# PinataFarms/FEARTracker

Measured on NVIDIA H100. Metric: FEAR-XS frames/sec (track + decode, batch 256 per GPU), higher is better.
Workload: dtype f32

## Files before the change

### feartracker_b200/csrc/kernels_tc.cuh

```cuda
#pragma once
#include <cuda_runtime.h>
#include <stdlib.h>

#include <initializer_list>

#include "tc_common.cuh"

namespace fear {
namespace tc {

constexpr int kCorrChunk = 32;
constexpr int kCorrABytes = 128 * 128;
constexpr int kCorrBBytes = 64 * 128;
constexpr int kTcThreads = 288;
constexpr int kTcConsumers = 256;

__device__ __forceinline__ void consumer_sync() { asm volatile("bar.sync 1, 256;" ::: "memory"); }

constexpr int kCorrStages = 3;
constexpr int kCorrStageBytes = kCorrABytes + 2 * kCorrBBytes;
constexpr int kCorrSmemBytes = kCorrStages * kCorrStageBytes + 1024  + 256 ;

__global__ void __launch_bounds__(kTcThreads, 1)
corr_tc_kernel(const __grid_constant__ CUtensorMap tmA, const __grid_constant__ CUtensorMap tmB,
               float* __restrict__ cat, int z_mod) {
  extern __shared__ uint8_t smem_raw[];
  uint8_t* smem = smem_raw + ((1024u - (smem_u32(smem_raw) & 1023u)) & 1023u);
  uint64_t* full = reinterpret_cast<uint64_t*>(smem + kCorrStages * kCorrStageBytes);
  uint64_t* empty = full + kCorrStages;
  const int warp = threadIdx.x >> 5, lane = threadIdx.x & 31;
  constexpr int kChunks = 256 / kCorrChunk;
  if (threadIdx.x == 0) {
    prefetch_tmap(&tmA);
    prefetch_tmap(&tmB);
    for (int s = 0; s < kCorrStages; ++s) {
      mbar_init(&full[s], 1);
      mbar_init(&empty[s], 8);
    }
    fence_mbar_init();
  }
  __syncthreads();
  pdl_trigger();
  pdl_wait();
  const int frame = blockIdx.x >> 1, half = blockIdx.x & 1;
  const int arow = frame * 256 + half * 128;
  auto st_x = [&](int s) { return smem + s * kCorrStageBytes; };
  auto st_z = [&](int s) { return smem + s * kCorrStageBytes + kCorrABytes; };

  if (warp == 8) {
    if (lane == 0) {
      const int brow = z_mod ? (frame % z_mod) * 64 : 0;
      for (int c = 0; c < kChunks; ++c) {
        const int stage = c % kCorrStages;
        mbar_wait_backoff(&empty[stage], (uint32_t)(((c / kCorrStages) & 1) ^ 1));
        mbar_arrive_expect_tx(&full[stage], kCorrABytes + kCorrBBytes);
        tma_load_2d(st_x(stage), &tmA, &full[stage], c * kCorrChunk, arow);
        tma_load_2d(st_z(stage), &tmB, &full[stage], c * kCorrChunk, brow);
      }
    }
    return;
  }
  const int wg = warp >> 2, r0 = wg * 64 + (warp & 3) * 16 + (lane >> 2), t = lane & 3;
  float accm[32], accc[32];
#pragma unroll
  for (int i = 0; i < 32; ++i) accm[i] = accc[i] = 0.f;
  for (int c = 0; c < kChunks; ++c) {
    const int stage = c % kCorrStages;
    mbar_wait(&full[stage], (uint32_t)((c / kCorrStages) & 1));
    float4* zh = reinterpret_cast<float4*>(st_z(stage));
    float4* zl = reinterpret_cast<float4*>(st_z(stage) + kCorrBBytes);
#pragma unroll
    for (int i = 0; i < kCorrBBytes / 16 / kTcConsumers; ++i) {
      const float4 v = zh[threadIdx.x + i * kTcConsumers];
      float4 h, l;
      split_tf32_trunc(v.x, h.x, l.x);
      split_tf32_trunc(v.y, h.y, l.y);
      split_tf32_trunc(v.z, h.z, l.z);
      split_tf32_trunc(v.w, h.w, l.w);
      zh[threadIdx.x + i * kTcConsumers] = h;
      zl[threadIdx.x + i * kTcConsumers] = l;
    }
    fence_proxy_async_smem();
    consumer_sync();
    uint32_t hi[4][4], lo[4][4];
    load_a_frags(st_x(stage), r0, t, hi, lo);
    const uint32_t bh = smem_u32(zh), bl = smem_u32(zl);
    wg_fence();
#pragma unroll
    for (int j = 0; j < 4; ++j) mma3<64>(accm, accc, hi[j], lo[j], bh + j * 32, bl + j * 32);
    wg_commit();
    wg_wait();
    __syncwarp();
    if (lane == 0) mbar_arrive(&empty[stage]);
  }
  float* out = cat + (long long)(arow + r0) * 320 + 256 + 2 * t;
#pragma unroll
  for (int i = 0; i < 8; ++i) {
    *reinterpret_cast<float2*>(out + 8 * i) = make_float2(accm[4 * i] + accc[4 * i], accm[4 * i + 1] + accc[4 * i + 1]);
    *reinterpret_cast<float2*>(out + 8 * 320 + 8 * i) =
        make_float2(accm[4 * i + 2] + accc[4 * i + 2], accm[4 * i + 3] + accc[4 * i + 3]);
  }
}

inline int init_pw();

inline int init() {
  int dev = 0;
  if (cudaGetDevice(&dev) != cudaSuccess) return -1;
  cudaDeviceProp p;
  if (cudaGetDeviceProperties(&p, dev) != cudaSuccess) return -1;
  DeviceState& st = dev_state();
  st.num_sms = p.multiProcessorCount;
  st.inited = true;
  if (resolve_driver()) return 0;
  if (cudaFuncSetAttribute(corr_tc_kernel, cudaFuncAttributeMaxDynamicSharedMemorySize, kCorrSmemBytes) != cudaSuccess) {
    cudaGetLastError();
    return 0;
  }
  if (init_pw()) return 0;
  st.tc_ready = true;
  return 0;
}

inline int launch_corr(cudaStream_t s, const float* zt, int Bz, float* cat, int B, int groups) {
  if (!available()) return -20;
  CUtensorMap tmA, tmB;
  const int frames = B * groups;
  int r;
  r = make_tmap_2d(&tmA, cat, (uint64_t)frames * 256, 320, 320, 128, kCorrChunk);
  if (r) return r;
  r = make_tmap_2d(&tmB, zt, (uint64_t)Bz * 64, 256, 256, 64, kCorrChunk);
  if (r) return r;
  if (launch_pdl(corr_tc_kernel, dim3(frames * 2), dim3(kTcThreads), kCorrSmemBytes, s, tmA, tmB, cat, Bz == 1 ? 0 : B) !=
      cudaSuccess)
    return -23;
  return 0;
}

struct PwParams {
  const float* bias;
  const float* R;
  float* C;
  int ldr, ldc;
  int M, N, num_n_tiles, num_tiles, num_chunks, last_ksteps, relu, stages, stage_bytes;
  int dw_relu, dw_bias;
  int box_bytes;
};

constexpr int kPwThreads = 384;
constexpr int kPwProducerRegs = 40, kPwConsumerRegs = 232;

template <int NT, int KS>
__device__ __forceinline__ void mma3_chunk(float* accm, float* accc, const uint32_t (&hi)[4][4], const uint32_t (&lo)[4][4],
                                           uint32_t bh, uint32_t bl) {
#pragma unroll
  for (int j = 0; j < KS; ++j) mma3<NT>(accm, accc, hi[j], lo[j], bh + j * 32, bl + j * 32);
}

template <int K, int MW>
__device__ __forceinline__ void dw_chunk(const uint8_t* box, const uint8_t* wts, const uint8_t* bia, uint8_t* at, int ct,
                                         int dw_bias, int dw_relu) {
  constexpr int TX = 8, NIN = TX + K - 1, IW = MW + K - 1, PXN = MW / TX;
  typedef unsigned long long U2;
  const int c2 = ct & 15, pos = ct >> 4;
  const int x0 = (pos % PXN) * TX, y0 = pos / PXN;
  const U2* in2 = reinterpret_cast<const U2*>(box) + (y0 * IW + x0) * 16 + c2;
  const U2* w2 = reinterpret_cast<const U2*>(wts) + c2;
  const U2 bias2 = dw_bias ? reinterpret_cast<const U2*>(bia)[c2] : 0ull;
  U2 acc[TX];
#pragma unroll
  for (int i = 0; i < TX; ++i) acc[i] = bias2;
#pragma unroll
  for (int ky = 0; ky < K; ++ky) {
    U2 v[NIN];
#pragma unroll
    for (int i = 0; i < NIN; ++i) v[i] = in2[(ky * IW + i) * 16];
#pragma unroll
    for (int kx = 0; kx < K; ++kx) {
      const U2 k = w2[(ky * K + kx) * 16];
#pragma unroll
      for (int i = 0; i < TX; ++i) ffma2(acc[i], v[i + kx], k);
    }
  }
#pragma unroll
  for (int i = 0; i < TX; ++i) {
    float2 v = make_float2(__uint_as_float((uint32_t)acc[i]), __uint_as_float((uint32_t)(acc[i] >> 32)));
    if (dw_relu) {
      v.x = fmaxf(v.x, 0.f);
      v.y = fmaxf(v.y, 0.f);
    }
    const int R = y0 * MW + x0 + i;
    *reinterpret_cast<float2*>(at + R * 128 + (((c2 >> 1) ^ (R & 7)) << 4) + ((c2 & 1) << 3)) = v;
  }
}

template <int NT>
__device__ __forceinline__ void pw_epilogue(const PwParams& p, const float* accm, const float* accc, int mt, int nt, int r0,
                                            int t) {
  const int n0 = nt * NT + 2 * t;
#pragma unroll
  for (int hrow = 0; hrow < 2; ++hrow) {
    const long long grow = (long long)mt * 128 + r0 + hrow * 8;
    if (grow >= p.M) continue;
#pragma unroll
    for (int i = 0; i < NT / 8; ++i) {
      const int col = n0 + 8 * i;
      if (col >= p.N) continue;
      float2 o = make_float2(accm[4 * i + 2 * hrow] + accc[4 * i + 2 * hrow], accm[4 * i + 2 * hrow + 1] + accc[4 * i + 2 * hrow + 1]);
      float2 b = p.bias ? __ldg(reinterpret_cast<const float2*>(p.bias + col)) : make_float2(0.f, 0.f);
      if (p.R) {
        const float2 rr = __ldg(reinterpret_cast<const float2*>(p.R + grow * p.ldr + col));
        b.x += rr.x;
        b.y += rr.y;
      }
      o.x += b.x;
      o.y += b.y;
      if (p.relu) {
        o.x = fmaxf(o.x, 0.f);
        o.y = fmaxf(o.y, 0.f);
      }
      *reinterpret_cast<float2*>(p.C + grow * p.ldc + col) = o;
    }
  }
}

template <int NT, int DWK, int MW = 16>
__global__ void __launch_bounds__(kPwThreads, 1)
pw_tc_kernel(const __grid_constant__ CUtensorMap tmA, const __grid_constant__ CUtensorMap tmWh,
             const __grid_constant__ CUtensorMap tmWl, const __grid_constant__ CUtensorMap tmDW,
             const __grid_constant__ CUtensorMap tmDB, const PwParams p) {
  extern __shared__ uint8_t smem_raw[];
  uint8_t* smem = smem_raw + ((1024u - (smem_u32(smem_raw) & 1023u)) & 1023u);
  const int S = p.stages;
  constexpr int a_bufs = DWK > 0 ? 2 : 0;
  uint64_t* full = reinterpret_cast<uint64_t*>(smem + S * p.stage_bytes + a_bufs * kCorrABytes);
  uint64_t* empty = full + S;
  constexpr int w_bytes = NT * 128;
  if (threadIdx.x == 0) {
    prefetch_tmap(&tmA);
    prefetch_tmap(&tmWh);
    prefetch_tmap(&tmWl);
    for (int s = 0; s < S; ++s) {
      mbar_init(&full[s], 1);
      mbar_init(&empty[s], 8);
    }
    fence_mbar_init();
  }
  __syncthreads();
  pdl_trigger();
  pdl_wait();

  auto a_tile = [&](int s) { return smem + s * p.stage_bytes; };
  auto a_buf = [&](int b) { return smem + S * p.stage_bytes + b * kCorrABytes; };
  auto w_hi = [&](int s) { return smem + s * p.stage_bytes + (DWK > 0 ? 0 : kCorrABytes); };
  auto w_lo = [&](int s) { return w_hi(s) + w_bytes; };
  auto dw_box = [&](int s) { return w_lo(s) + w_bytes; };
  auto dw_wts = [&](int s) { return dw_box(s) + p.box_bytes; };
  auto dw_bia = [&](int s) { return dw_wts(s) + DWK * DWK * 128; };

  const int wg = __shfl_sync(0xffffffffu, (int)threadIdx.x / 128, 0);
  if (wg == 0) {
    setmaxnreg_dec<kPwProducerRegs>();
    if (threadIdx.x == 0) {
      constexpr int th = 128 / MW, tpf = MW / th;
      int stage = 0;
      uint32_t phase = 0;
      for (int tile = blockIdx.x; tile < p.num_tiles; tile += gridDim.x) {
        const int mt = tile / p.num_n_tiles, nt = tile - mt * p.num_n_tiles;
        for (int c = 0; c < p.num_chunks; ++c) {
          mbar_wait_backoff(&empty[stage], phase ^ 1);
          if constexpr (DWK > 0) {
            mbar_arrive_expect_tx(&full[stage], 2 * w_bytes + p.box_bytes + DWK * DWK * 128 + (p.dw_bias ? 128 : 0));
            tma_load_4d(dw_box(stage), &tmA, &full[stage], c * 32, -(DWK / 2), (mt % tpf) * th - DWK / 2, mt / tpf);
            tma_load_2d(dw_wts(stage), &tmDW, &full[stage], c * 32, 0);
            if (p.dw_bias) tma_load_2d(dw_bia(stage), &tmDB, &full[stage], c * 32, 0);
          } else {
            mbar_arrive_expect_tx(&full[stage], kCorrABytes + 2 * w_bytes);
            tma_load_2d(a_tile(stage), &tmA, &full[stage], c * 32, mt * 128);
          }
          tma_load_2d(w_hi(stage), &tmWh, &full[stage], c * 32, nt * NT);
          tma_load_2d(w_lo(stage), &tmWl, &full[stage], c * 32, nt * NT);
          if (++stage == S) {
            stage = 0;
            phase ^= 1;
          }
        }
      }
    }
    return;
  }
  setmaxnreg_inc<kPwConsumerRegs>();

  const int ct = threadIdx.x - 128, warp = ct >> 5, lane = ct & 31;
  const int r0 = (warp >> 2) * 64 + (warp & 3) * 16 + (lane >> 2), t = lane & 3;
  int stage = 0, ab = 0;
  uint32_t phase = 0;
  for (int tile = blockIdx.x; tile < p.num_tiles; tile += gridDim.x) {
    const int mt = tile / p.num_n_tiles, nt = tile - mt * p.num_n_tiles;
    float accm[NT / 2], accc[NT / 2];
#pragma unroll
    for (int i = 0; i < NT / 2; ++i) accm[i] = accc[i] = 0.f;
    if constexpr (DWK > 0) {
      mbar_wait(&full[stage], phase);
      dw_chunk<DWK, MW>(dw_box(stage), dw_wts(stage), dw_bia(stage), a_buf(ab), ct, p.dw_bias, p.dw_relu);
      consumer_sync();
    }
    int prev = 0;
    for (int c = 0; c < p.num_chunks; ++c) {
      if constexpr (DWK == 0) mbar_wait(&full[stage], phase);
      uint32_t hi[4][4], lo[4][4];
      load_a_frags(DWK > 0 ? a_buf(ab) : a_tile(stage), r0, t, hi, lo);
      const uint32_t bh = smem_u32(w_hi(stage)), bl = smem_u32(w_lo(stage));
      const int ksteps = (c == p.num_chunks - 1) ? p.last_ksteps : 4;
      wg_fence();
      if (ksteps == 4) mma3_chunk<NT, 4>(accm, accc, hi, lo, bh, bl);
      else if (ksteps == 3) mma3_chunk<NT, 3>(accm, accc, hi, lo, bh, bl);
      else if (ksteps == 2) mma3_chunk<NT, 2>(accm, accc, hi, lo, bh, bl);
      else mma3_chunk<NT, 1>(accm, accc, hi, lo, bh, bl);
      wg_commit();
      if (c > 0) {
        wg_wait_n<1>();
        __syncwarp();
        if (lane == 0) mbar_arrive(&empty[prev]);
      }
      prev = stage;
      if (++stage == S) {
        stage = 0;
        phase ^= 1;
      }
      if constexpr (DWK > 0) {
        ab ^= 1;
        if (c + 1 < p.num_chunks) {
          mbar_wait(&full[stage], phase);
          dw_chunk<DWK, MW>(dw_box(stage), dw_wts(stage), dw_bia(stage), a_buf(ab), ct, p.dw_bias, p.dw_relu);
          consumer_sync();
        }
      }
    }
    wg_wait_n<0>();
    __syncwarp();
    if (lane == 0) mbar_arrive(&empty[prev]);
    pw_epilogue<NT>(p, accm, accc, mt, nt, r0, t);
  }
}

template <int NT>
__global__ void __launch_bounds__(kTcThreads, 1)
pw_tc_narrow_kernel(const __grid_constant__ CUtensorMap tmA, const __grid_constant__ CUtensorMap tmWh,
                    const __grid_constant__ CUtensorMap tmWl, const PwParams p) {
  extern __shared__ uint8_t smem_raw[];
  uint8_t* smem = smem_raw + ((1024u - (smem_u32(smem_raw) & 1023u)) & 1023u);
  const int S = p.stages;
  uint64_t* full = reinterpret_cast<uint64_t*>(smem + S * p.stage_bytes);
  uint64_t* empty = full + S;
  const int warp = threadIdx.x >> 5, lane = threadIdx.x & 31;
  constexpr int w_bytes = NT * 128;
  if (threadIdx.x == 0) {
    prefetch_tmap(&tmA);
    prefetch_tmap(&tmWh);
    prefetch_tmap(&tmWl);
    for (int s = 0; s < S; ++s) {
      mbar_init(&full[s], 1);
      mbar_init(&empty[s], 8);
    }
    fence_mbar_init();
  }
  __syncthreads();
  pdl_trigger();
  pdl_wait();

  const int mt = blockIdx.x / p.num_n_tiles, nt = blockIdx.x - mt * p.num_n_tiles;
  auto a_tile = [&](int s) { return smem + s * p.stage_bytes; };
  auto w_hi = [&](int s) { return smem + s * p.stage_bytes + kCorrABytes; };
  auto w_lo = [&](int s) { return w_hi(s) + w_bytes; };

  if (warp == 8) {
    if (lane == 0) {
      for (int c = 0; c < p.num_chunks; ++c) {
        const int stage = c % S;
        mbar_wait_backoff(&empty[stage], (uint32_t)(((c / S) & 1) ^ 1));
        mbar_arrive_expect_tx(&full[stage], kCorrABytes + 2 * w_bytes);
        tma_load_2d(a_tile(stage), &tmA, &full[stage], c * 32, mt * 128);
        tma_load_2d(w_hi(stage), &tmWh, &full[stage], c * 32, nt * NT);
        tma_load_2d(w_lo(stage), &tmWl, &full[stage], c * 32, nt * NT);
      }
    }
    return;
  }

  const int wg = warp >> 2, r0 = wg * 64 + (warp & 3) * 16 + (lane >> 2), t = lane & 3;
  float accm[NT / 2], accc[NT / 2];
#pragma unroll
  for (int i = 0; i < NT / 2; ++i) accm[i] = accc[i] = 0.f;
  for (int c = 0; c < p.num_chunks; ++c) {
    const int stage = c % S;
    mbar_wait(&full[stage], (uint32_t)((c / S) & 1));
    uint32_t hi[4][4], lo[4][4];
    load_a_frags(a_tile(stage), r0, t, hi, lo);
    const uint32_t bh = smem_u32(w_hi(stage)), bl = smem_u32(w_lo(stage));
    const int ksteps = (c == p.num_chunks - 1) ? p.last_ksteps : 4;
    wg_fence();
#pragma unroll
    for (int j = 0; j < 4; ++j)
      if (j < ksteps) mma3<NT>(accm, accc, hi[j], lo[j], bh + j * 32, bl + j * 32);
    wg_commit();
    wg_wait();
    __syncwarp();
    if (lane == 0) mbar_arrive(&empty[stage]);
  }
  pw_epilogue<NT>(p, accm, accc, mt, nt, r0, t);
}

constexpr int kPwMaxSmem = 232448 - 1024;
constexpr int kPwMaxStages = 4;
constexpr int kPwSmemExtra = 1024  + 256 ;

inline int pw_stages(int stage_bytes, int fixed_bytes) {
  const int fit = (kPwMaxSmem - kPwSmemExtra - fixed_bytes) / stage_bytes;
  return fit < kPwMaxStages ? fit : kPwMaxStages;
}

inline int pw_tile_n(int N) {
  const int Np = (N + 15) & ~15;
  const int tiles = (Np + 127) / 128;
  const int need = (Np + tiles - 1) / tiles;
  for (int nt : {16, 32, 48, 64, 96, 112, 128})
    if (nt >= need) return nt;
  return 0;
}

inline bool pw_supported(int cin, int cout) { return available() && cin % 8 == 0 && cout % 8 == 0; }

#define FEAR_PW_FOR_NT(X) X(16) X(32) X(48) X(64) X(96) X(112) X(128)

constexpr int kPwNarrowNT = 32;
inline int pw_tile_n_one_chunk(int N) {
  const int Np = (N + 15) & ~15;
  const int tiles = (Np + kPwNarrowNT - 1) / kPwNarrowNT;
  const int need = (Np + tiles - 1) / tiles;
  return need <= 16 ? 16 : 32;
}

inline int init_pw() {
  cudaError_t e = cudaSuccess;
#define FEAR_PW_ATTR(NT_)                                                                                                  \
  if (e == cudaSuccess) e = cudaFuncSetAttribute(pw_tc_kernel<NT_, 0>, cudaFuncAttributeMaxDynamicSharedMemorySize, kPwMaxSmem);     \
  if (e == cudaSuccess) e = cudaFuncSetAttribute(pw_tc_kernel<NT_, 3, 16>, cudaFuncAttributeMaxDynamicSharedMemorySize, kPwMaxSmem); \
  if (e == cudaSuccess) e = cudaFuncSetAttribute(pw_tc_kernel<NT_, 5, 16>, cudaFuncAttributeMaxDynamicSharedMemorySize, kPwMaxSmem); \
  if (e == cudaSuccess) e = cudaFuncSetAttribute(pw_tc_kernel<NT_, 3, 32>, cudaFuncAttributeMaxDynamicSharedMemorySize, kPwMaxSmem); \
  if (e == cudaSuccess) e = cudaFuncSetAttribute(pw_tc_kernel<NT_, 5, 32>, cudaFuncAttributeMaxDynamicSharedMemorySize, kPwMaxSmem);
  FEAR_PW_FOR_NT(FEAR_PW_ATTR)
#undef FEAR_PW_ATTR
  if (e == cudaSuccess) e = cudaFuncSetAttribute(pw_tc_narrow_kernel<16>, cudaFuncAttributeMaxDynamicSharedMemorySize, kPwMaxSmem);
  if (e == cudaSuccess) e = cudaFuncSetAttribute(pw_tc_narrow_kernel<32>, cudaFuncAttributeMaxDynamicSharedMemorySize, kPwMaxSmem);
  if (e != cudaSuccess) {
    cudaGetLastError();
    return -1;
  }
  return 0;
}

inline dim3 pw_grid(int tiles) { return dim3(tiles < num_sms() ? tiles : num_sms()); }

inline int launch_pw(cudaStream_t s, const float* A, int lda, const float* w_hi, const float* w_lo, const float* bias,
                     const float* R, int ldr, float* C, int ldc, int M, int N, int K, int relu) {
  if (!available()) return -20;
  PwParams p;
  p.bias = bias;
  p.R = R;
  p.C = C;
  p.ldr = ldr;
  p.ldc = ldc;
  p.M = M;
  p.N = N;
  p.num_chunks = (K + 31) / 32;
  const bool narrow = p.num_chunks == 1;
  const int NT = narrow ? pw_tile_n_one_chunk(N) : pw_tile_n(N);
  if (!NT) return -21;
  p.num_n_tiles = (((N + 15) & ~15) + NT - 1) / NT;
  p.num_tiles = ((M + 127) / 128) * p.num_n_tiles;
  p.last_ksteps = ((K - 32 * (p.num_chunks - 1)) + 7) / 8;
  p.relu = relu;
  p.dw_relu = p.dw_bias = p.box_bytes = 0;
  p.stage_bytes = kCorrABytes + 2 * NT * 128;
  p.stages = narrow ? 1 : pw_stages(p.stage_bytes, 0);
  CUtensorMap tmA, tmWh, tmWl;
  int r = make_tmap_2d(&tmA, A, (uint64_t)M, (uint64_t)K, (uint64_t)lda, 128, 32);
  if (r) return r;
  r = make_tmap_2d(&tmWh, w_hi, (uint64_t)N, (uint64_t)K, (uint64_t)K, NT, 32);
  if (r) return r;
  r = make_tmap_2d(&tmWl, w_lo, (uint64_t)N, (uint64_t)K, (uint64_t)K, NT, 32);
  if (r) return r;
  const size_t smem_bytes = (size_t)p.stages * p.stage_bytes + kPwSmemExtra;
  cudaError_t e = cudaErrorInvalidValue;
  if (narrow) {
    if (NT == 16) e = launch_pdl(pw_tc_narrow_kernel<16>, dim3(p.num_tiles), dim3(kTcThreads), smem_bytes, s, tmA, tmWh, tmWl, p);
    else e = launch_pdl(pw_tc_narrow_kernel<32>, dim3(p.num_tiles), dim3(kTcThreads), smem_bytes, s, tmA, tmWh, tmWl, p);
    return e == cudaSuccess ? 0 : -23;
  }
  switch (NT) {
#define FEAR_PW_CASE(NT_)                                                                                               \
  case NT_:                                                                                                             \
    e = launch_pdl(pw_tc_kernel<NT_, 0>, pw_grid(p.num_tiles), dim3(kPwThreads), smem_bytes, s, tmA, tmWh, tmWl, tmA, tmA, p); \
    break;
    FEAR_PW_FOR_NT(FEAR_PW_CASE)
#undef FEAR_PW_CASE
  }
  return e == cudaSuccess ? 0 : -23;
}

inline int launch_pw_dw(cudaStream_t s, const float* X, int B, int dw_k, const float* dw_w, const float* dw_b, int dw_relu,
                        const float* w_hi, const float* w_lo, const float* bias, const float* R, int ldr, float* C,
                        int ldc, int N, int K, int relu, int map_w = 16) {
  if (!available()) return -20;
  if ((dw_k != 3 && dw_k != 5) || K % 4 || (map_w != 16 && map_w != 32)) return 1;
  PwParams p;
  const int M = B * map_w * map_w;
  p.bias = bias;
  p.R = R;
  p.C = C;
  p.ldr = ldr;
  p.ldc = ldc;
  p.M = M;
  p.N = N;
  p.num_chunks = (K + 31) / 32;
  const int NT = pw_tile_n(N);
  if (!NT) return 1;
  p.num_n_tiles = (((N + 15) & ~15) + NT - 1) / NT;
  p.num_tiles = (M / 128) * p.num_n_tiles;
  p.last_ksteps = ((K - 32 * (p.num_chunks - 1)) + 7) / 8;
  p.relu = relu;
  p.dw_relu = dw_relu;
  p.dw_bias = dw_b != nullptr;
  const int ih = 128 / map_w + dw_k - 1, iw = map_w + dw_k - 1;
  p.box_bytes = ih * iw * 128;
  p.stage_bytes = (2 * NT * 128 + p.box_bytes + dw_k * dw_k * 128 + 128 + 1023) & ~1023;
  if ((p.num_chunks < 2 ? 1 : 2) * (kCorrABytes + p.stage_bytes) + kPwSmemExtra > kPwMaxSmem) return 1;
  p.stages = pw_stages(p.stage_bytes, 2 * kCorrABytes);
  const size_t smem_bytes = (size_t)p.stages * p.stage_bytes + 2 * kCorrABytes + kPwSmemExtra;
  CUtensorMap tmX, tmWh, tmWl, tmDW, tmDB;
  int r = make_tmap_nhwc(&tmX, X, (uint64_t)B, (uint64_t)map_w, (uint64_t)map_w, (uint64_t)K, 32, iw, ih);
  if (r) return r;
  r = make_tmap_2d(&tmWh, w_hi, (uint64_t)N, (uint64_t)K, (uint64_t)K, NT, 32);
  if (r) return r;
  r = make_tmap_2d(&tmWl, w_lo, (uint64_t)N, (uint64_t)K, (uint64_t)K, NT, 32);
  if (r) return r;
  r = make_tmap_2d_plain(&tmDW, dw_w, (uint64_t)dw_k * dw_k, (uint64_t)K, dw_k * dw_k, 32);
  if (r) return r;
  if (dw_b) {
    r = make_tmap_2d_plain(&tmDB, dw_b, 1, (uint64_t)K, 1, 32);
    if (r) return r;
  } else {
    tmDB = tmDW;
  }
  cudaError_t e = cudaErrorInvalidValue;
#define FEAR_PW_DW_LAUNCH(NT_, K_, MW_) \
  e = launch_pdl(pw_tc_kernel<NT_, K_, MW_>, pw_grid(p.num_tiles), dim3(kPwThreads), smem_bytes, s, tmX, tmWh, tmWl, tmDW, tmDB, p)
  switch (NT) {
#define FEAR_PW_CASE(NT_)                                \
  case NT_:                                              \
    if (map_w == 16) {                                   \
      if (dw_k == 5) FEAR_PW_DW_LAUNCH(NT_, 5, 16);      \
      else FEAR_PW_DW_LAUNCH(NT_, 3, 16);                \
    } else {                                             \
      if (dw_k == 5) FEAR_PW_DW_LAUNCH(NT_, 5, 32);      \
      else FEAR_PW_DW_LAUNCH(NT_, 3, 32);                \
    }                                                    \
    break;
    FEAR_PW_FOR_NT(FEAR_PW_CASE)
#undef FEAR_PW_CASE
  }
#undef FEAR_PW_DW_LAUNCH
  return e == cudaSuccess ? 0 : -23;
}

}
}
```

Before: 36370.

## Stage pointwise GEMM epilogue through swizzled shared memory and store via TMA

Adds a TMA-store epilogue to the pointwise tensor-core kernel. Accumulators get bias, residual and ReLU applied, are written into double-buffered swizzled shared-memory slabs, and are stored with bulk tensor stores instead of per-thread float2 global writes. This aims to make output writes coalesced and asynchronous so they can overlap the next tile. In exchange the plain GEMM path reserves two extra staging buffers of shared memory, which can reduce the ring stage count, and it adds named-barrier syncs and store drains per tile.

```diff
diff --git a/feartracker_b200/csrc/kernels_tc.cuh b/feartracker_b200/csrc/kernels_tc.cuh
--- a/feartracker_b200/csrc/kernels_tc.cuh
+++ b/feartracker_b200/csrc/kernels_tc.cuh
@@ -145,6 +145,7 @@
   int M, N, num_n_tiles, num_tiles, num_chunks, last_ksteps, relu, stages, stage_bytes;
   int dw_relu, dw_bias;
   int box_bytes;
+  int tma_store;
 };
 
 constexpr int kPwThreads = 384;
@@ -224,22 +225,87 @@
   }
 }
 
+constexpr int kPwSlabBytes = 64 * 128;
+constexpr int kPwBoxBytes = 64 * 64;
+template <int NT>
+__host__ __device__ constexpr int pw_slabs() { return (NT + 31) / 32; }
+
+__device__ __forceinline__ void wg_sync(int wgc) { asm volatile("bar.sync %0, 128;" ::"r"(2 + wgc) : "memory"); }
+
+template <int NT>
+__device__ __forceinline__ void pw_epilogue_tma(const PwParams& p, const CUtensorMap* tmC, float* accm, const float* accc,
+                                                int mt, int nt, int wgc, int wr, int t, uint8_t* last, uint8_t* other,
+                                                bool leader) {
+  const long long row0 = (long long)mt * 128 + wgc * 64;
+#pragma unroll
+  for (int i = 0; i < NT / 8; ++i) {
+    const int col = nt * NT + 8 * i + 2 * t;
+#pragma unroll
+    for (int hrow = 0; hrow < 2; ++hrow) {
+      const long long grow = row0 + wr + hrow * 8;
+      float2 o = make_float2(accm[4 * i + 2 * hrow] + accc[4 * i + 2 * hrow], accm[4 * i + 2 * hrow + 1] + accc[4 * i + 2 * hrow + 1]);
+      if (grow < p.M && col < p.N) {
+        float2 b = p.bias ? __ldg(reinterpret_cast<const float2*>(p.bias + col)) : make_float2(0.f, 0.f);
+        if (p.R) {
+          const float2 rr = __ldg(reinterpret_cast<const float2*>(p.R + grow * p.ldr + col));
+          b.x += rr.x;
+          b.y += rr.y;
+        }
+        o.x += b.x;
+        o.y += b.y;
+      }
+      if (p.relu) {
+        o.x = fmaxf(o.x, 0.f);
+        o.y = fmaxf(o.y, 0.f);
+      }
+      accm[4 * i + 2 * hrow] = o.x;
+      accm[4 * i + 2 * hrow + 1] = o.y;
+    }
+  }
+#pragma unroll
+  for (int s = 0; s < pw_slabs<NT>(); ++s) {
+    uint8_t* buf = (pw_slabs<NT>() - 1 - s) & 1 ? other : last;
+    if (leader) tma_store_wait_read<1>();
+    wg_sync(wgc);
+#pragma unroll
+    for (int i = 4 * s; i < 4 * s + 4 && i < NT / 8; ++i) {
+      const int cc = 8 * (i & 1) + 2 * t;
+#pragma unroll
+      for (int hrow = 0; hrow < 2; ++hrow) {
+        const int r = wr + hrow * 8;
+        *reinterpret_cast<float2*>(buf + ((i >> 1) & 1) * kPwBoxBytes + r * 64 + (((cc >> 2) ^ ((r >> 1) & 3)) << 4) +
+                                   (cc & 3) * 4) = make_float2(accm[4 * i + 2 * hrow], accm[4 * i + 2 * hrow + 1]);
+      }
+    }
+    fence_proxy_async_smem();
+    wg_sync(wgc);
+    if (leader) {
+#pragma unroll
+      for (int b = 0; b < 2 && 32 * s + 16 * b < NT; ++b) {
+        const int col0 = nt * NT + 32 * s + 16 * b;
+        if (col0 < p.N && row0 < p.M) tma_store_2d(tmC, buf + b * kPwBoxBytes, col0, (int)row0);
+      }
+      tma_store_commit();
+    }
+  }
+}
+
 template <int NT, int DWK, int MW = 16>
 __global__ void __launch_bounds__(kPwThreads, 1)
 pw_tc_kernel(const __grid_constant__ CUtensorMap tmA, const __grid_constant__ CUtensorMap tmWh,
              const __grid_constant__ CUtensorMap tmWl, const __grid_constant__ CUtensorMap tmDW,
-             const __grid_constant__ CUtensorMap tmDB, const PwParams p) {
+             const __grid_constant__ CUtensorMap tmDB, const __grid_constant__ CUtensorMap tmC, const PwParams p) {
   extern __shared__ uint8_t smem_raw[];
   uint8_t* smem = smem_raw + ((1024u - (smem_u32(smem_raw) & 1023u)) & 1023u);
   const int S = p.stages;
-  constexpr int a_bufs = DWK > 0 ? 2 : 0;
-  uint64_t* full = reinterpret_cast<uint64_t*>(smem + S * p.stage_bytes + a_bufs * kCorrABytes);
+  uint64_t* full = reinterpret_cast<uint64_t*>(smem + S * p.stage_bytes + 2 * kCorrABytes);
   uint64_t* empty = full + S;
   constexpr int w_bytes = NT * 128;
   if (threadIdx.x == 0) {
     prefetch_tmap(&tmA);
     prefetch_tmap(&tmWh);
     prefetch_tmap(&tmWl);
+    if (p.tma_store) prefetch_tmap(&tmC);
     for (int s = 0; s < S; ++s) {
       mbar_init(&full[s], 1);
       mbar_init(&empty[s], 8);
@@ -292,17 +358,26 @@
   setmaxnreg_inc<kPwConsumerRegs>();
 
   const int ct = threadIdx.x - 128, warp = ct >> 5, lane = ct & 31;
-  const int r0 = (warp >> 2) * 64 + (warp & 3) * 16 + (lane >> 2), t = lane & 3;
+  const int wgc = warp >> 2, wr = (warp & 3) * 16 + (lane >> 2), t = lane & 3;
+  const int r0 = wgc * 64 + wr;
+  const bool leader = (ct & 127) == 0;
   int stage = 0, ab = 0;
   uint32_t phase = 0;
+  int slab = 0;
   for (int tile = blockIdx.x; tile < p.num_tiles; tile += gridDim.x) {
     const int mt = tile / p.num_n_tiles, nt = tile - mt * p.num_n_tiles;
     float accm[NT / 2], accc[NT / 2];
 #pragma unroll
     for (int i = 0; i < NT / 2; ++i) accm[i] = accc[i] = 0.f;
     if constexpr (DWK > 0) {
+      const bool drain = p.tma_store && tile != blockIdx.x;
+      if (drain) {
+        if (leader) tma_store_wait_read<1>();
+        consumer_sync();
+      }
       mbar_wait(&full[stage], phase);
       dw_chunk<DWK, MW>(dw_box(stage), dw_wts(stage), dw_bia(stage), a_buf(ab), ct, p.dw_bias, p.dw_relu);
+      if (drain && leader) tma_store_wait_read<0>();
       consumer_sync();
     }
     int prev = 0;
@@ -340,8 +415,15 @@
     wg_wait_n<0>();
     __syncwarp();
     if (lane == 0) mbar_arrive(&empty[prev]);
-    pw_epilogue<NT>(p, accm, accc, mt, nt, r0, t);
-  }
+    if (p.tma_store) {
+      const int lb = DWK > 0 ? ab ^ 1 : (slab + pw_slabs<NT>() - 1) & 1;
+      slab += pw_slabs<NT>();
+      pw_epilogue_tma<NT>(p, &tmC, accm, accc, mt, nt, wgc, wr, t, a_buf(lb) + wgc * kPwSlabBytes,
+                          a_buf(lb ^ 1) + wgc * kPwSlabBytes, leader);
+    } else
+      pw_epilogue<NT>(p, accm, accc, mt, nt, r0, t);
+  }
+  if (leader && p.tma_store) tma_store_wait<0>();
 }
 
 template <int NT>
@@ -418,6 +500,15 @@
 inline int pw_stages(int stage_bytes, int fixed_bytes) {
   const int fit = (kPwMaxSmem - kPwSmemExtra - fixed_bytes) / stage_bytes;
   return fit < kPwMaxStages ? fit : kPwMaxStages;
+}
+
+constexpr int kPwStagingBytes = 2 * kCorrABytes;
+static_assert(kPwMaxStages * (kCorrABytes + 2 * 128 * 128) + kPwStagingBytes + kPwSmemExtra <= kPwMaxSmem,
+              "pw_tc_kernel<128, 0>: four ring stages and the staging buffers fit in shared memory");
+
+inline int make_tmap_out(CUtensorMap* m, float* C, int ldc, int M, int N) {
+  if ((reinterpret_cast<uintptr_t>(C) & 15) || (ldc & 3)) return 1;
+  return make_tmap_2d(m, C, (uint64_t)M, (uint64_t)N, (uint64_t)ldc, 64, 16);
 }
 
 inline int pw_tile_n(int N) {
@@ -481,9 +572,9 @@
   p.num_tiles = ((M + 127) / 128) * p.num_n_tiles;
   p.last_ksteps = ((K - 32 * (p.num_chunks - 1)) + 7) / 8;
   p.relu = relu;
-  p.dw_relu = p.dw_bias = p.box_bytes = 0;
+  p.dw_relu = p.dw_bias = p.box_bytes = p.tma_store = 0;
   p.stage_bytes = kCorrABytes + 2 * NT * 128;
-  p.stages = narrow ? 1 : pw_stages(p.stage_bytes, 0);
+  p.stages = narrow ? 1 : pw_stages(p.stage_bytes, kPwStagingBytes);
   CUtensorMap tmA, tmWh, tmWl;
   int r = make_tmap_2d(&tmA, A, (uint64_t)M, (uint64_t)K, (uint64_t)lda, 128, 32);
   if (r) return r;
@@ -491,17 +582,23 @@
   if (r) return r;
   r = make_tmap_2d(&tmWl, w_lo, (uint64_t)N, (uint64_t)K, (uint64_t)K, NT, 32);
   if (r) return r;
-  const size_t smem_bytes = (size_t)p.stages * p.stage_bytes + kPwSmemExtra;
   cudaError_t e = cudaErrorInvalidValue;
   if (narrow) {
+    const size_t smem_bytes = (size_t)p.stages * p.stage_bytes + kPwSmemExtra;
     if (NT == 16) e = launch_pdl(pw_tc_narrow_kernel<16>, dim3(p.num_tiles), dim3(kTcThreads), smem_bytes, s, tmA, tmWh, tmWl, p);
     else e = launch_pdl(pw_tc_narrow_kernel<32>, dim3(p.num_tiles), dim3(kTcThreads), smem_bytes, s, tmA, tmWh, tmWl, p);
     return e == cudaSuccess ? 0 : -23;
   }
+  CUtensorMap tmC = tmA;
+  r = make_tmap_out(&tmC, C, ldc, M, N);
+  if (r < 0) return r;
+  p.tma_store = r == 0;
+  const size_t smem_bytes = (size_t)p.stages * p.stage_bytes + kPwStagingBytes + kPwSmemExtra;
   switch (NT) {
 #define FEAR_PW_CASE(NT_)                                                                                               \
   case NT_:                                                                                                             \
-    e = launch_pdl(pw_tc_kernel<NT_, 0>, pw_grid(p.num_tiles), dim3(kPwThreads), smem_bytes, s, tmA, tmWh, tmWl, tmA, tmA, p); \
+    e = launch_pdl(pw_tc_kernel<NT_, 0>, pw_grid(p.num_tiles), dim3(kPwThreads), smem_bytes, s, tmA, tmWh, tmWl, tmA, tmA, \
+                   tmC, p);                                                                                             \
     break;
     FEAR_PW_FOR_NT(FEAR_PW_CASE)
 #undef FEAR_PW_CASE
@@ -538,7 +635,7 @@
   if ((p.num_chunks < 2 ? 1 : 2) * (kCorrABytes + p.stage_bytes) + kPwSmemExtra > kPwMaxSmem) return 1;
   p.stages = pw_stages(p.stage_bytes, 2 * kCorrABytes);
   const size_t smem_bytes = (size_t)p.stages * p.stage_bytes + 2 * kCorrABytes + kPwSmemExtra;
-  CUtensorMap tmX, tmWh, tmWl, tmDW, tmDB;
+  CUtensorMap tmX, tmWh, tmWl, tmDW, tmDB, tmC;
   int r = make_tmap_nhwc(&tmX, X, (uint64_t)B, (uint64_t)map_w, (uint64_t)map_w, (uint64_t)K, 32, iw, ih);
   if (r) return r;
   r = make_tmap_2d(&tmWh, w_hi, (uint64_t)N, (uint64_t)K, (uint64_t)K, NT, 32);
@@ -553,9 +650,14 @@
   } else {
     tmDB = tmDW;
   }
+  tmC = tmX;
+  r = NT > 32 ? make_tmap_out(&tmC, C, ldc, M, N) : 1;
+  if (r < 0) return r;
+  p.tma_store = r == 0;
   cudaError_t e = cudaErrorInvalidValue;
-#define FEAR_PW_DW_LAUNCH(NT_, K_, MW_) \
-  e = launch_pdl(pw_tc_kernel<NT_, K_, MW_>, pw_grid(p.num_tiles), dim3(kPwThreads), smem_bytes, s, tmX, tmWh, tmWl, tmDW, tmDB, p)
+#define FEAR_PW_DW_LAUNCH(NT_, K_, MW_)                                                                              \
+  e = launch_pdl(pw_tc_kernel<NT_, K_, MW_>, pw_grid(p.num_tiles), dim3(kPwThreads), smem_bytes, s, tmX, tmWh, tmWl, \
+                 tmDW, tmDB, tmC, p)
   switch (NT) {
 #define FEAR_PW_CASE(NT_)                                \
   case NT_:                                              \
```

After: 38940, median of 6. 1.07x the previous value.
